# CPJKU/beat_this

Hardware: NVIDIA H100
Metric: clips/sec (30 s audio->beats, final0) (higher is better)
Workload: dtype f16

## Files before the change

beat_this_b200/csrc/kernels_attn.cu:

```cuda
#include <cstdio>

#include "tc_common.cuh"

namespace bt {

constexpr int AT_BQ = 128;
constexpr int AT_BKV = 64;
constexpr int AT_NST = 4;
constexpr int AT_WARPS = 8;
constexpr int AT_THREADS = 32 * (AT_WARPS + 1);
constexpr int AT_SQ = AT_BQ * 64;
constexpr int AT_SKV = AT_BKV * 64;
constexpr int AT_SMEM = 1024 + AT_SQ + AT_NST * 2 * AT_SKV + 128;

constexpr uint32_t AT_POLY_MASK = 0x52u;

__device__ __forceinline__ uint32_t sw64_off(int r, int c) {
  return static_cast<uint32_t>(r * 64 + ((c ^ ((r >> 1) & 3)) << 4));
}

__global__ void __launch_bounds__(AT_THREADS, 2)
attn_time_kernel(const __grid_constant__ CUtensorMap tmQ, const __grid_constant__ CUtensorMap tmKV,
                 const float* __restrict__ gates, h16* __restrict__ out, int L, int heads,
                 const ChunkSrc* __restrict__ chunks, int seqs_per_chunk) {
  extern __shared__ uint8_t smem_raw[];
  const uint32_t sbase = (smem_u32(smem_raw) + 1023u) & ~1023u;
  const uint32_t sQ = sbase;
  const uint32_t sK = sQ + AT_SQ;
  const uint32_t sV = sK + AT_NST * AT_SKV;
  const uint32_t bar_q = sV + AT_NST * AT_SKV;
  const uint32_t full = bar_q + 8;
  const uint32_t empty = full + 8 * AT_NST;

  const int warp = threadIdx.x >> 5, lane = threadIdx.x & 31;
  const int q0 = blockIdx.x * AT_BQ;
  const int h = blockIdx.y;
  const int seq = blockIdx.z;
  const int C = heads * 32;
  const int Lk = chunks ? chunks[seq / seqs_per_chunk].len : L;
  const int nkv = ceil_div(Lk, AT_BKV);

  if (threadIdx.x == 0) {
    mbar_init(bar_q, 1);
    for (int i = 0; i < AT_NST; ++i) {
      mbar_init(full + 8 * i, 1);
      mbar_init(empty + 8 * i, AT_WARPS);
    }
    fence_barrier_init();
  }
  __syncthreads();

  if (warp == AT_WARPS) {
    if (lane == 0) {
      tma_prefetch_desc(&tmQ);
      tma_prefetch_desc(&tmKV);
      mbar_expect_tx(bar_q, AT_SQ);
      tma_load_3d(sQ, &tmQ, bar_q, h * 32, q0, seq);
      for (int j = 0; j < nkv; ++j) {
        const int st = j % AT_NST;
        if (j >= AT_NST) mbar_wait(empty + 8 * st, ((j / AT_NST) - 1) & 1);
        mbar_expect_tx(full + 8 * st, 2 * AT_SKV);
        tma_load_3d(sK + st * AT_SKV, &tmKV, full + 8 * st, C + h * 32, j * AT_BKV, seq);
        tma_load_3d(sV + st * AT_SKV, &tmKV, full + 8 * st, 2 * C + h * 32, j * AT_BKV, seq);
      }
    }
    return;
  }

  const int r0 = warp * 16;
  mbar_wait(bar_q, 0);
  uint32_t qa[2][4];
#pragma unroll
  for (int ks = 0; ks < 2; ++ks) ldmatrix_x4(sQ + sw64_off(r0 + (lane & 15), 2 * ks + (lane >> 4)), qa[ks]);

  float o[4][4];
#pragma unroll
  for (int d = 0; d < 4; ++d) o[d][0] = o[d][1] = o[d][2] = o[d][3] = 0.f;
  float m_run[2] = {-INFINITY, -INFINITY}, l_run[2] = {0.f, 0.f};
  for (int j = 0; j < nkv; ++j) {
    const int st = j % AT_NST;
    mbar_wait(full + 8 * st, (j / AT_NST) & 1);
    const uint32_t kb = sK + st * AT_SKV, vb = sV + st * AT_SKV;
    float s[8][4];
#pragma unroll
    for (int nb = 0; nb < 8; ++nb) {
      s[nb][0] = s[nb][1] = s[nb][2] = s[nb][3] = 0.f;
      uint32_t kf[4];
      ldmatrix_x4(kb + sw64_off(nb * 8 + (lane & 7), lane >> 3), kf);
      mma_16816(s[nb], qa[0], kf[0], kf[1]);
      mma_16816(s[nb], qa[1], kf[2], kf[3]);
    }
    if (j == nkv - 1) {
      const int lim = Lk - j * AT_BKV;
#pragma unroll
      for (int nb = 0; nb < 8; ++nb) {
        const int key = nb * 8 + 2 * (lane & 3);
        if (key >= lim) s[nb][0] = s[nb][2] = -INFINITY;
        if (key + 1 >= lim) s[nb][1] = s[nb][3] = -INFINITY;
      }
    }
    float mx[2] = {-INFINITY, -INFINITY};
#pragma unroll
    for (int nb = 0; nb < 8; ++nb) {
      mx[0] = fmaxf(mx[0], fmaxf(s[nb][0], s[nb][1]));
      mx[1] = fmaxf(mx[1], fmaxf(s[nb][2], s[nb][3]));
    }
    float mref[2], alpha[2];
#pragma unroll
    for (int r = 0; r < 2; ++r) {
      mx[r] = fmaxf(mx[r], __shfl_xor_sync(0xffffffffu, mx[r], 1));
      mx[r] = fmaxf(mx[r], __shfl_xor_sync(0xffffffffu, mx[r], 2));
      mref[r] = fmaxf(m_run[r], mx[r]);
      alpha[r] = ex2_approx(m_run[r] - mref[r]);
      m_run[r] = mref[r];
      l_run[r] *= alpha[r];
    }
#pragma unroll
    for (int d = 0; d < 4; ++d) {
      o[d][0] *= alpha[0]; o[d][1] *= alpha[0];
      o[d][2] *= alpha[1]; o[d][3] *= alpha[1];
    }
    uint32_t pa[4][4];
#pragma unroll
    for (int nb = 0; nb < 8; ++nb) {
      float p[4];
#pragma unroll
      for (int i = 0; i < 4; ++i) {
        const float x = s[nb][i] - mref[i >> 1];
        p[i] = ((AT_POLY_MASK >> nb) & 1u) ? ex2_poly(x) : ex2_approx(x);
      }
      l_run[0] += p[0] + p[1];
      l_run[1] += p[2] + p[3];
      pa[nb >> 1][(nb & 1) * 2] = pack_h16x2(p[0], p[1]);
      pa[nb >> 1][(nb & 1) * 2 + 1] = pack_h16x2(p[2], p[3]);
    }
#pragma unroll
    for (int kk = 0; kk < 4; ++kk) {
      const int key = kk * 16 + (lane & 7) + ((lane >> 3) & 1) * 8;
#pragma unroll
      for (int dp = 0; dp < 2; ++dp) {
        uint32_t vf[4];
        ldmatrix_x4_trans(vb + sw64_off(key, 2 * dp + (lane >> 4)), vf);
        mma_16816(o[2 * dp], pa[kk], vf[0], vf[1]);
        mma_16816(o[2 * dp + 1], pa[kk], vf[2], vf[3]);
      }
    }
    __syncwarp();
    if (lane == 0) mbar_arrive(empty + 8 * st);
  }
#pragma unroll
  for (int r = 0; r < 2; ++r) {
    l_run[r] += __shfl_xor_sync(0xffffffffu, l_run[r], 1);
    l_run[r] += __shfl_xor_sync(0xffffffffu, l_run[r], 2);
  }
#pragma unroll
  for (int r = 0; r < 2; ++r) {
    const int q = q0 + r0 + (lane >> 2) + 8 * r;
    if (q < L) {
      const int64_t m = static_cast<int64_t>(seq) * L + q;
      const float gsc = gates[m * heads + h] / l_run[r];
      h16* dst = out + m * C + h * 32 + 2 * (lane & 3);
#pragma unroll
      for (int d = 0; d < 4; ++d)
        *reinterpret_cast<uint32_t*>(dst + 8 * d) = pack_h16x2(o[d][2 * r] * gsc, o[d][2 * r + 1] * gsc);
    }
  }
}

struct TcAttnPlan {
  CUtensorMap tmQ;
  CUtensorMap tmKV;
  int seqs, L, heads;
};

TcAttnPlan* tc_attn_plan_create(const void* qkv, int seqs, int L, int heads, char* err, int errlen) {
  TcAttnPlan* p = new TcAttnPlan();
  p->seqs = seqs; p->L = L; p->heads = heads;
  const int C = heads * 32;
  const uint64_t dims[3] = {static_cast<uint64_t>(3 * C), static_cast<uint64_t>(L), static_cast<uint64_t>(seqs)};
  const uint64_t strides[2] = {static_cast<uint64_t>(3 * C) * 2, static_cast<uint64_t>(L) * 3 * C * 2};
  const uint32_t box_q[3] = {32, AT_BQ, 1};
  const uint32_t box_kv[3] = {32, AT_BKV, 1};
  if (!make_tmap(&p->tmQ, qkv, 3, dims, strides, box_q, 64, err, errlen) ||
      !make_tmap(&p->tmKV, qkv, 3, dims, strides, box_kv, 64, err, errlen)) {
    delete p;
    return nullptr;
  }
  return p;
}
void tc_attn_plan_destroy(TcAttnPlan* p) { delete p; }

void launch_attn_time_tc(const TcAttnPlan* p, const float* gates, void* out, cudaStream_t st, const ChunkSrc* chunks,
                         int seqs_per_chunk) {
  dim3 grid(ceil_div(p->L, AT_BQ), p->heads, p->seqs);
  attn_time_kernel<<<grid, AT_THREADS, AT_SMEM, st>>>(p->tmQ, p->tmKV, gates, reinterpret_cast<h16*>(out), p->L, p->heads,
                                                      chunks, seqs_per_chunk);
}

int tc_init_attn(char* err, int errlen) {
  const cudaError_t r = cudaFuncSetAttribute(attn_time_kernel, cudaFuncAttributeMaxDynamicSharedMemorySize, AT_SMEM);
  if (r != cudaSuccess) {
    snprintf(err, errlen, "cudaFuncSetAttribute(attn_time_kernel) failed: %s", cudaGetErrorString(r));
    return -1;
  }
  return 0;
}

}
```

Baseline: 746.4.

## Fold TMA producer into consumer thread and peel masked last KV tile

Removes the dedicated producer warp. Thread 0 of the first consumer warp issues the initial KV prefetches, then refills each stage one iteration late after waiting on the empty barrier. The loop body moves into a templated tile function: the boundary mask applies only to the peeled final tile, the running max uses a tree reduction, ldmatrix addresses are precomputed per lane, and output rescaling is skipped when alpha is one for the whole warp. Dropping the producer warp frees warp slots and registers, but refill latency now sits on a compute warp's critical path and that warp may stall waiting for the others to release a stage.

```diff
diff --git a/beat_this_b200/csrc/kernels_attn.cu b/beat_this_b200/csrc/kernels_attn.cu
--- a/beat_this_b200/csrc/kernels_attn.cu
+++ b/beat_this_b200/csrc/kernels_attn.cu
@@ -8,7 +8,7 @@
 constexpr int AT_BKV = 64;
 constexpr int AT_NST = 4;
 constexpr int AT_WARPS = 8;
-constexpr int AT_THREADS = 32 * (AT_WARPS + 1);
+constexpr int AT_THREADS = 32 * AT_WARPS;
 constexpr int AT_SQ = AT_BQ * 64;
 constexpr int AT_SKV = AT_BKV * 64;
 constexpr int AT_SMEM = 1024 + AT_SQ + AT_NST * 2 * AT_SKV + 128;
@@ -17,6 +17,86 @@
 
 __device__ __forceinline__ uint32_t sw64_off(int r, int c) {
   return static_cast<uint32_t>(r * 64 + ((c ^ ((r >> 1) & 3)) << 4));
+}
+
+__device__ __forceinline__ uint32_t opaque_u32(uint32_t v) {
+  asm volatile("" : "+r"(v));
+  return v;
+}
+
+template <bool kMasked>
+__device__ __forceinline__ void attn_time_tile(const uint32_t (&qa)[2][4], uint32_t kaddr, uint32_t vaddr, int key0,
+                                               int lim, float (&o)[4][4], float (&m_run)[2], float (&l_run)[2]) {
+  float s[8][4];
+#pragma unroll
+  for (int nb = 0; nb < 8; ++nb) {
+    s[nb][0] = s[nb][1] = s[nb][2] = s[nb][3] = 0.f;
+    uint32_t kf[4];
+    ldmatrix_x4(kaddr + nb * 8 * 64, kf);
+    mma_16816(s[nb], qa[0], kf[0], kf[1]);
+    mma_16816(s[nb], qa[1], kf[2], kf[3]);
+  }
+  if constexpr (kMasked) {
+#pragma unroll
+    for (int nb = 0; nb < 8; ++nb) {
+      const int key = nb * 8 + key0;
+      if (key >= lim) s[nb][0] = s[nb][2] = -INFINITY;
+      if (key + 1 >= lim) s[nb][1] = s[nb][3] = -INFINITY;
+    }
+  }
+  float mref[2], alpha[2];
+#pragma unroll
+  for (int r = 0; r < 2; ++r) {
+    float t[8];
+#pragma unroll
+    for (int nb = 0; nb < 8; ++nb) t[nb] = fmaxf(s[nb][2 * r], s[nb][2 * r + 1]);
+#pragma unroll
+    for (int w = 4; w > 0; w >>= 1)
+#pragma unroll
+      for (int i = 0; i < w; ++i) t[i] = fmaxf(t[i], t[i + w]);
+    float mx = fmaxf(t[0], __shfl_xor_sync(0xffffffffu, t[0], 1));
+    mx = fmaxf(mx, __shfl_xor_sync(0xffffffffu, mx, 2));
+    mref[r] = fmaxf(m_run[r], mx);
+    alpha[r] = ex2_approx(m_run[r] - mref[r]);
+    m_run[r] = mref[r];
+  }
+  if (!__all_sync(0xffffffffu, alpha[0] == 1.f && alpha[1] == 1.f)) {
+#pragma unroll
+    for (int d = 0; d < 4; ++d) {
+      o[d][0] *= alpha[0]; o[d][1] *= alpha[0];
+      o[d][2] *= alpha[1]; o[d][3] *= alpha[1];
+    }
+  }
+#pragma unroll
+  for (int kk = 0; kk < 4; ++kk) {
+    uint32_t pa[4];
+#pragma unroll
+    for (int h = 0; h < 2; ++h) {
+      const int nb = 2 * kk + h;
+      float p[4];
+#pragma unroll
+      for (int i = 0; i < 4; ++i) {
+        const float x = s[nb][i] - mref[i >> 1];
+        p[i] = ((AT_POLY_MASK >> nb) & 1u) ? ex2_poly(x) : ex2_approx(x);
+      }
+      if (nb == 0) {
+        l_run[0] = fmaf(l_run[0], alpha[0], p[0] + p[1]);
+        l_run[1] = fmaf(l_run[1], alpha[1], p[2] + p[3]);
+      } else {
+        l_run[0] += p[0] + p[1];
+        l_run[1] += p[2] + p[3];
+      }
+      pa[2 * h] = pack_h16x2(p[0], p[1]);
+      pa[2 * h + 1] = pack_h16x2(p[2], p[3]);
+    }
+#pragma unroll
+    for (int dp = 0; dp < 2; ++dp) {
+      uint32_t vf[4];
+      ldmatrix_x4_trans((vaddr ^ (dp * 32)) + kk * 16 * 64, vf);
+      mma_16816(o[2 * dp], pa, vf[0], vf[1]);
+      mma_16816(o[2 * dp + 1], pa, vf[2], vf[3]);
+    }
+  }
 }
 
 __global__ void __launch_bounds__(AT_THREADS, 2)
@@ -39,115 +119,59 @@
   const int C = heads * 32;
   const int Lk = chunks ? chunks[seq / seqs_per_chunk].len : L;
   const int nkv = ceil_div(Lk, AT_BKV);
-
-  if (threadIdx.x == 0) {
+  const bool producer = threadIdx.x == 0;
+  auto load_kv = [&](int t) {
+    const int st = t % AT_NST;
+    mbar_expect_tx(full + 8 * st, 2 * AT_SKV);
+    tma_load_3d(sK + st * AT_SKV, &tmKV, full + 8 * st, C + h * 32, t * AT_BKV, seq);
+    tma_load_3d(sV + st * AT_SKV, &tmKV, full + 8 * st, 2 * C + h * 32, t * AT_BKV, seq);
+  };
+
+  if (producer) {
     mbar_init(bar_q, 1);
     for (int i = 0; i < AT_NST; ++i) {
       mbar_init(full + 8 * i, 1);
       mbar_init(empty + 8 * i, AT_WARPS);
     }
     fence_barrier_init();
+    tma_prefetch_desc(&tmQ);
+    tma_prefetch_desc(&tmKV);
+    mbar_expect_tx(bar_q, AT_SQ);
+    tma_load_3d(sQ, &tmQ, bar_q, h * 32, q0, seq);
+    for (int t = 0; t < AT_NST && t < nkv; ++t) load_kv(t);
   }
   __syncthreads();
-
-  if (warp == AT_WARPS) {
-    if (lane == 0) {
-      tma_prefetch_desc(&tmQ);
-      tma_prefetch_desc(&tmKV);
-      mbar_expect_tx(bar_q, AT_SQ);
-      tma_load_3d(sQ, &tmQ, bar_q, h * 32, q0, seq);
-      for (int j = 0; j < nkv; ++j) {
-        const int st = j % AT_NST;
-        if (j >= AT_NST) mbar_wait(empty + 8 * st, ((j / AT_NST) - 1) & 1);
-        mbar_expect_tx(full + 8 * st, 2 * AT_SKV);
-        tma_load_3d(sK + st * AT_SKV, &tmKV, full + 8 * st, C + h * 32, j * AT_BKV, seq);
-        tma_load_3d(sV + st * AT_SKV, &tmKV, full + 8 * st, 2 * C + h * 32, j * AT_BKV, seq);
-      }
-    }
-    return;
-  }
 
   const int r0 = warp * 16;
   mbar_wait(bar_q, 0);
   uint32_t qa[2][4];
 #pragma unroll
   for (int ks = 0; ks < 2; ++ks) ldmatrix_x4(sQ + sw64_off(r0 + (lane & 15), 2 * ks + (lane >> 4)), qa[ks]);
+  const uint32_t kaddr = opaque_u32(sK + sw64_off(lane & 7, lane >> 3));
+  const uint32_t vaddr = opaque_u32(sV + sw64_off(lane & 15, lane >> 4));
+  const int key0 = 2 * (lane & 3);
 
   float o[4][4];
 #pragma unroll
   for (int d = 0; d < 4; ++d) o[d][0] = o[d][1] = o[d][2] = o[d][3] = 0.f;
   float m_run[2] = {-INFINITY, -INFINITY}, l_run[2] = {0.f, 0.f};
-  for (int j = 0; j < nkv; ++j) {
-    const int st = j % AT_NST;
+  const uint32_t nrefill = opaque_u32(producer && nkv > AT_NST ? nkv - AT_NST : 0);
+  const int nsteady = static_cast<int>(opaque_u32(nkv - 1));
+  for (int j = 0; j < nsteady; ++j) {
+    const uint32_t st = j % AT_NST, so = st * AT_SKV;
     mbar_wait(full + 8 * st, (j / AT_NST) & 1);
-    const uint32_t kb = sK + st * AT_SKV, vb = sV + st * AT_SKV;
-    float s[8][4];
-#pragma unroll
-    for (int nb = 0; nb < 8; ++nb) {
-      s[nb][0] = s[nb][1] = s[nb][2] = s[nb][3] = 0.f;
-      uint32_t kf[4];
-      ldmatrix_x4(kb + sw64_off(nb * 8 + (lane & 7), lane >> 3), kf);
-      mma_16816(s[nb], qa[0], kf[0], kf[1]);
-      mma_16816(s[nb], qa[1], kf[2], kf[3]);
-    }
-    if (j == nkv - 1) {
-      const int lim = Lk - j * AT_BKV;
-#pragma unroll
-      for (int nb = 0; nb < 8; ++nb) {
-        const int key = nb * 8 + 2 * (lane & 3);
-        if (key >= lim) s[nb][0] = s[nb][2] = -INFINITY;
-        if (key + 1 >= lim) s[nb][1] = s[nb][3] = -INFINITY;
-      }
-    }
-    float mx[2] = {-INFINITY, -INFINITY};
-#pragma unroll
-    for (int nb = 0; nb < 8; ++nb) {
-      mx[0] = fmaxf(mx[0], fmaxf(s[nb][0], s[nb][1]));
-      mx[1] = fmaxf(mx[1], fmaxf(s[nb][2], s[nb][3]));
-    }
-    float mref[2], alpha[2];
-#pragma unroll
-    for (int r = 0; r < 2; ++r) {
-      mx[r] = fmaxf(mx[r], __shfl_xor_sync(0xffffffffu, mx[r], 1));
-      mx[r] = fmaxf(mx[r], __shfl_xor_sync(0xffffffffu, mx[r], 2));
-      mref[r] = fmaxf(m_run[r], mx[r]);
-      alpha[r] = ex2_approx(m_run[r] - mref[r]);
-      m_run[r] = mref[r];
-      l_run[r] *= alpha[r];
-    }
-#pragma unroll
-    for (int d = 0; d < 4; ++d) {
-      o[d][0] *= alpha[0]; o[d][1] *= alpha[0];
-      o[d][2] *= alpha[1]; o[d][3] *= alpha[1];
-    }
-    uint32_t pa[4][4];
-#pragma unroll
-    for (int nb = 0; nb < 8; ++nb) {
-      float p[4];
-#pragma unroll
-      for (int i = 0; i < 4; ++i) {
-        const float x = s[nb][i] - mref[i >> 1];
-        p[i] = ((AT_POLY_MASK >> nb) & 1u) ? ex2_poly(x) : ex2_approx(x);
-      }
-      l_run[0] += p[0] + p[1];
-      l_run[1] += p[2] + p[3];
-      pa[nb >> 1][(nb & 1) * 2] = pack_h16x2(p[0], p[1]);
-      pa[nb >> 1][(nb & 1) * 2 + 1] = pack_h16x2(p[2], p[3]);
-    }
-#pragma unroll
-    for (int kk = 0; kk < 4; ++kk) {
-      const int key = kk * 16 + (lane & 7) + ((lane >> 3) & 1) * 8;
-#pragma unroll
-      for (int dp = 0; dp < 2; ++dp) {
-        uint32_t vf[4];
-        ldmatrix_x4_trans(vb + sw64_off(key, 2 * dp + (lane >> 4)), vf);
-        mma_16816(o[2 * dp], pa[kk], vf[0], vf[1]);
-        mma_16816(o[2 * dp + 1], pa[kk], vf[2], vf[3]);
-      }
-    }
-    __syncwarp();
+    attn_time_tile<false>(qa, kaddr + so, vaddr + so, key0, 0, o, m_run, l_run);
+    if (static_cast<uint32_t>(j - 1) < nrefill) {
+      const int t = j + AT_NST - 1;
+      mbar_wait(empty + 8 * (t % AT_NST), ((t / AT_NST) - 1) & 1);
+      load_kv(t);
+    }
     if (lane == 0) mbar_arrive(empty + 8 * st);
   }
+  const uint32_t st = nsteady % AT_NST, parity = (nsteady / AT_NST) & 1;
+  mbar_wait(full + 8 * st, parity);
+  const uint32_t so = st * AT_SKV;
+  attn_time_tile<true>(qa, kaddr + so, vaddr + so, key0, Lk - nsteady * AT_BKV, o, m_run, l_run);
 #pragma unroll
   for (int r = 0; r < 2; ++r) {
     l_run[r] += __shfl_xor_sync(0xffffffffu, l_run[r], 1);
```

Result: faster. 766.2 (median of 6 runs) (+2.7%).

## Give each attention warp two query row blocks and drop the producer warp

Applied to the files above, without the earlier changes.

The time-attention kernel now runs 4 warps, each handling two 16-row query blocks, so every K and V ldmatrix fragment feeds twice as many MMAs. The dedicated TMA producer warp is removed: thread 0 issues the initial stages and refills the ring inline, waiting on the previous stage's empty barrier. The last-tile masking is split into a compile-time specialised step, shared-memory addresses are precomputed, and launch bounds target 3 blocks per SM. This raises register pressure per thread, and refilling from a consumer thread can stall that warp's compute.

```diff
diff --git a/beat_this_b200/csrc/kernels_attn.cu b/beat_this_b200/csrc/kernels_attn.cu
--- a/beat_this_b200/csrc/kernels_attn.cu
+++ b/beat_this_b200/csrc/kernels_attn.cu
@@ -1,4 +1,5 @@
 #include <cstdio>
+#include <type_traits>
 
 #include "tc_common.cuh"
 
@@ -7,11 +8,13 @@
 constexpr int AT_BQ = 128;
 constexpr int AT_BKV = 64;
 constexpr int AT_NST = 4;
-constexpr int AT_WARPS = 8;
-constexpr int AT_THREADS = 32 * (AT_WARPS + 1);
+constexpr int AT_WARPS = 4;
+constexpr int AT_RB = 2;
+constexpr int AT_THREADS = 32 * AT_WARPS;
 constexpr int AT_SQ = AT_BQ * 64;
 constexpr int AT_SKV = AT_BKV * 64;
 constexpr int AT_SMEM = 1024 + AT_SQ + AT_NST * 2 * AT_SKV + 128;
+static_assert(AT_BQ == AT_WARPS * AT_RB * 16, "every query row of the tile belongs to one row block");
 
 constexpr uint32_t AT_POLY_MASK = 0x52u;
 
@@ -19,7 +22,7 @@
   return static_cast<uint32_t>(r * 64 + ((c ^ ((r >> 1) & 3)) << 4));
 }
 
-__global__ void __launch_bounds__(AT_THREADS, 2)
+__global__ void __launch_bounds__(AT_THREADS, 3)
 attn_time_kernel(const __grid_constant__ CUtensorMap tmQ, const __grid_constant__ CUtensorMap tmKV,
                  const float* __restrict__ gates, h16* __restrict__ out, int L, int heads,
                  const ChunkSrc* __restrict__ chunks, int seqs_per_chunk) {
@@ -50,121 +53,163 @@
   }
   __syncthreads();
 
-  if (warp == AT_WARPS) {
-    if (lane == 0) {
-      tma_prefetch_desc(&tmQ);
-      tma_prefetch_desc(&tmKV);
-      mbar_expect_tx(bar_q, AT_SQ);
-      tma_load_3d(sQ, &tmQ, bar_q, h * 32, q0, seq);
-      for (int j = 0; j < nkv; ++j) {
-        const int st = j % AT_NST;
-        if (j >= AT_NST) mbar_wait(empty + 8 * st, ((j / AT_NST) - 1) & 1);
-        mbar_expect_tx(full + 8 * st, 2 * AT_SKV);
-        tma_load_3d(sK + st * AT_SKV, &tmKV, full + 8 * st, C + h * 32, j * AT_BKV, seq);
-        tma_load_3d(sV + st * AT_SKV, &tmKV, full + 8 * st, 2 * C + h * 32, j * AT_BKV, seq);
-      }
-    }
-    return;
-  }
-
-  const int r0 = warp * 16;
+  auto load_tile = [&](int t) {
+    const int st = t % AT_NST;
+    mbar_expect_tx(full + 8 * st, 2 * AT_SKV);
+    tma_load_3d(sK + st * AT_SKV, &tmKV, full + 8 * st, C + h * 32, t * AT_BKV, seq);
+    tma_load_3d(sV + st * AT_SKV, &tmKV, full + 8 * st, 2 * C + h * 32, t * AT_BKV, seq);
+  };
+  if (threadIdx.x == 0) {
+    tma_prefetch_desc(&tmQ);
+    tma_prefetch_desc(&tmKV);
+    mbar_expect_tx(bar_q, AT_SQ);
+    tma_load_3d(sQ, &tmQ, bar_q, h * 32, q0, seq);
+    for (int t = 0; t < nkv && t < AT_NST; ++t) load_tile(t);
+  }
+
+  const int r0 = warp * (AT_RB * 16);
   mbar_wait(bar_q, 0);
-  uint32_t qa[2][4];
-#pragma unroll
-  for (int ks = 0; ks < 2; ++ks) ldmatrix_x4(sQ + sw64_off(r0 + (lane & 15), 2 * ks + (lane >> 4)), qa[ks]);
-
-  float o[4][4];
-#pragma unroll
-  for (int d = 0; d < 4; ++d) o[d][0] = o[d][1] = o[d][2] = o[d][3] = 0.f;
-  float m_run[2] = {-INFINITY, -INFINITY}, l_run[2] = {0.f, 0.f};
-  for (int j = 0; j < nkv; ++j) {
-    const int st = j % AT_NST;
-    mbar_wait(full + 8 * st, (j / AT_NST) & 1);
-    const uint32_t kb = sK + st * AT_SKV, vb = sV + st * AT_SKV;
-    float s[8][4];
+
+  uint32_t qa[AT_RB][2][4];
+#pragma unroll
+  for (int b = 0; b < AT_RB; ++b)
+#pragma unroll
+    for (int ks = 0; ks < 2; ++ks)
+      ldmatrix_x4(sQ + sw64_off(r0 + 16 * b + (lane & 15), 2 * ks + (lane >> 4)), qa[b][ks]);
+
+  const uint32_t k_addr0 = sK + sw64_off(lane & 7, lane >> 3);
+  const uint32_t v_addr0[2] = {sV + sw64_off(lane & 15, lane >> 4), sV + sw64_off(lane & 15, 2 + (lane >> 4))};
+  const int key_lane = 2 * (lane & 3);
+
+  float o[AT_RB][4][4];
+#pragma unroll
+  for (int b = 0; b < AT_RB; ++b)
+#pragma unroll
+    for (int d = 0; d < 4; ++d) o[b][d][0] = o[b][d][1] = o[b][d][2] = o[b][d][3] = 0.f;
+  float m_run[AT_RB][2], l_run[AT_RB][2];
+#pragma unroll
+  for (int b = 0; b < AT_RB; ++b) m_run[b][0] = m_run[b][1] = -INFINITY, l_run[b][0] = l_run[b][1] = 0.f;
+  auto kv_step = [&](uint32_t stage, uint32_t phase, auto last, int lim) {
+    mbar_wait(full + stage / (AT_SKV / 8), phase);
+    const uint32_t ka = k_addr0 + stage, va0 = v_addr0[0] + stage, va1 = v_addr0[1] + stage;
+    float s[AT_RB][8][4];
 #pragma unroll
     for (int nb = 0; nb < 8; ++nb) {
-      s[nb][0] = s[nb][1] = s[nb][2] = s[nb][3] = 0.f;
       uint32_t kf[4];
-      ldmatrix_x4(kb + sw64_off(nb * 8 + (lane & 7), lane >> 3), kf);
-      mma_16816(s[nb], qa[0], kf[0], kf[1]);
-      mma_16816(s[nb], qa[1], kf[2], kf[3]);
-    }
-    if (j == nkv - 1) {
-      const int lim = Lk - j * AT_BKV;
+      ldmatrix_x4(ka + nb * 512, kf);
+#pragma unroll
+      for (int b = 0; b < AT_RB; ++b) {
+        s[b][nb][0] = s[b][nb][1] = s[b][nb][2] = s[b][nb][3] = 0.f;
+        mma_16816(s[b][nb], qa[b][0], kf[0], kf[1]);
+        mma_16816(s[b][nb], qa[b][1], kf[2], kf[3]);
+      }
+    }
+    if constexpr (decltype(last)::value) {
 #pragma unroll
       for (int nb = 0; nb < 8; ++nb) {
-        const int key = nb * 8 + 2 * (lane & 3);
-        if (key >= lim) s[nb][0] = s[nb][2] = -INFINITY;
-        if (key + 1 >= lim) s[nb][1] = s[nb][3] = -INFINITY;
-      }
-    }
-    float mx[2] = {-INFINITY, -INFINITY};
-#pragma unroll
-    for (int nb = 0; nb < 8; ++nb) {
-      mx[0] = fmaxf(mx[0], fmaxf(s[nb][0], s[nb][1]));
-      mx[1] = fmaxf(mx[1], fmaxf(s[nb][2], s[nb][3]));
-    }
-    float mref[2], alpha[2];
-#pragma unroll
-    for (int r = 0; r < 2; ++r) {
-      mx[r] = fmaxf(mx[r], __shfl_xor_sync(0xffffffffu, mx[r], 1));
-      mx[r] = fmaxf(mx[r], __shfl_xor_sync(0xffffffffu, mx[r], 2));
-      mref[r] = fmaxf(m_run[r], mx[r]);
-      alpha[r] = ex2_approx(m_run[r] - mref[r]);
-      m_run[r] = mref[r];
-      l_run[r] *= alpha[r];
-    }
-#pragma unroll
-    for (int d = 0; d < 4; ++d) {
-      o[d][0] *= alpha[0]; o[d][1] *= alpha[0];
-      o[d][2] *= alpha[1]; o[d][3] *= alpha[1];
-    }
-    uint32_t pa[4][4];
-#pragma unroll
-    for (int nb = 0; nb < 8; ++nb) {
-      float p[4];
-#pragma unroll
-      for (int i = 0; i < 4; ++i) {
-        const float x = s[nb][i] - mref[i >> 1];
-        p[i] = ((AT_POLY_MASK >> nb) & 1u) ? ex2_poly(x) : ex2_approx(x);
-      }
-      l_run[0] += p[0] + p[1];
-      l_run[1] += p[2] + p[3];
-      pa[nb >> 1][(nb & 1) * 2] = pack_h16x2(p[0], p[1]);
-      pa[nb >> 1][(nb & 1) * 2 + 1] = pack_h16x2(p[2], p[3]);
-    }
+        const int key = nb * 8 + key_lane;
+#pragma unroll
+        for (int b = 0; b < AT_RB; ++b) {
+          if (key >= lim) s[b][nb][0] = s[b][nb][2] = -INFINITY;
+          if (key + 1 >= lim) s[b][nb][1] = s[b][nb][3] = -INFINITY;
+        }
+      }
+    }
+    float mref[AT_RB][2];
+#pragma unroll
+    for (int b = 0; b < AT_RB; ++b) {
+      float mx[2];
+#pragma unroll
+      for (int r = 0; r < 2; ++r) {
+        float t[8];
+#pragma unroll
+        for (int nb = 0; nb < 8; ++nb) t[nb] = fmaxf(s[b][nb][2 * r], s[b][nb][2 * r + 1]);
+#pragma unroll
+        for (int w = 4; w > 0; w >>= 1)
+#pragma unroll
+          for (int i = 0; i < w; ++i) t[i] = fmaxf(t[i], t[i + w]);
+        mx[r] = t[0];
+      }
+      float alpha[2];
+#pragma unroll
+      for (int r = 0; r < 2; ++r) {
+        mx[r] = fmaxf(mx[r], __shfl_xor_sync(0xffffffffu, mx[r], 1));
+        mx[r] = fmaxf(mx[r], __shfl_xor_sync(0xffffffffu, mx[r], 2));
+        mref[b][r] = fmaxf(m_run[b][r], mx[r]);
+        alpha[r] = ex2_approx(m_run[b][r] - mref[b][r]);
+        m_run[b][r] = mref[b][r];
+        l_run[b][r] *= alpha[r];
+      }
+#pragma unroll
+      for (int d = 0; d < 4; ++d) {
+        o[b][d][0] *= alpha[0]; o[b][d][1] *= alpha[0];
+        o[b][d][2] *= alpha[1]; o[b][d][3] *= alpha[1];
+      }
+    }
+    uint32_t pa[AT_RB][4][4];
+#pragma unroll
+    for (int b = 0; b < AT_RB; ++b)
+#pragma unroll
+      for (int nb = 0; nb < 8; ++nb) {
+        float p[4];
+#pragma unroll
+        for (int i = 0; i < 4; ++i) {
+          const float x = s[b][nb][i] - mref[b][i >> 1];
+          p[i] = ((AT_POLY_MASK >> nb) & 1u) ? ex2_poly(x) : ex2_approx(x);
+        }
+        l_run[b][0] += p[0] + p[1];
+        l_run[b][1] += p[2] + p[3];
+        pa[b][nb >> 1][(nb & 1) * 2] = pack_h16x2(p[0], p[1]);
+        pa[b][nb >> 1][(nb & 1) * 2 + 1] = pack_h16x2(p[2], p[3]);
+      }
 #pragma unroll
     for (int kk = 0; kk < 4; ++kk) {
-      const int key = kk * 16 + (lane & 7) + ((lane >> 3) & 1) * 8;
 #pragma unroll
       for (int dp = 0; dp < 2; ++dp) {
         uint32_t vf[4];
-        ldmatrix_x4_trans(vb + sw64_off(key, 2 * dp + (lane >> 4)), vf);
-        mma_16816(o[2 * dp], pa[kk], vf[0], vf[1]);
-        mma_16816(o[2 * dp + 1], pa[kk], vf[2], vf[3]);
+        ldmatrix_x4_trans((dp ? va1 : va0) + kk * 1024, vf);
+#pragma unroll
+        for (int b = 0; b < AT_RB; ++b) {
+          mma_16816(o[b][2 * dp], pa[b][kk], vf[0], vf[1]);
+          mma_16816(o[b][2 * dp + 1], pa[b][kk], vf[2], vf[3]);
+        }
       }
     }
     __syncwarp();
-    if (lane == 0) mbar_arrive(empty + 8 * st);
-  }
-#pragma unroll
-  for (int r = 0; r < 2; ++r) {
-    l_run[r] += __shfl_xor_sync(0xffffffffu, l_run[r], 1);
-    l_run[r] += __shfl_xor_sync(0xffffffffu, l_run[r], 2);
-  }
-#pragma unroll
-  for (int r = 0; r < 2; ++r) {
-    const int q = q0 + r0 + (lane >> 2) + 8 * r;
-    if (q < L) {
-      const int64_t m = static_cast<int64_t>(seq) * L + q;
-      const float gsc = gates[m * heads + h] / l_run[r];
-      h16* dst = out + m * C + h * 32 + 2 * (lane & 3);
-#pragma unroll
-      for (int d = 0; d < 4; ++d)
-        *reinterpret_cast<uint32_t*>(dst + 8 * d) = pack_h16x2(o[d][2 * r] * gsc, o[d][2 * r + 1] * gsc);
-    }
-  }
+    if (lane == 0) mbar_arrive(empty + stage / (AT_SKV / 8));
+  };
+  uint32_t stage = 0, phase = 0;
+  for (int j = 0; j < nkv - 1; ++j) {
+    if (threadIdx.x == 0 && j > 0 && j + AT_NST - 1 < nkv) {
+      mbar_wait(empty + 8 * ((j - 1) % AT_NST), ((j - 1) / AT_NST) & 1);
+      load_tile(j + AT_NST - 1);
+    }
+    kv_step(stage, phase, std::false_type{}, 0);
+    stage += AT_SKV;
+    if (stage == AT_NST * AT_SKV) stage = 0, phase ^= 1;
+  }
+  if (nkv > 0) kv_step(stage, phase, std::true_type{}, Lk - (nkv - 1) * AT_BKV);
+#pragma unroll
+  for (int b = 0; b < AT_RB; ++b)
+#pragma unroll
+    for (int r = 0; r < 2; ++r) {
+      l_run[b][r] += __shfl_xor_sync(0xffffffffu, l_run[b][r], 1);
+      l_run[b][r] += __shfl_xor_sync(0xffffffffu, l_run[b][r], 2);
+    }
+#pragma unroll
+  for (int b = 0; b < AT_RB; ++b)
+#pragma unroll
+    for (int r = 0; r < 2; ++r) {
+      const int q = q0 + r0 + 16 * b + (lane >> 2) + 8 * r;
+      if (q < L) {
+        const int64_t m = static_cast<int64_t>(seq) * L + q;
+        const float gsc = gates[m * heads + h] / l_run[b][r];
+        h16* dst = out + m * C + h * 32 + 2 * (lane & 3);
+#pragma unroll
+        for (int d = 0; d < 4; ++d)
+          *reinterpret_cast<uint32_t*>(dst + 8 * d) = pack_h16x2(o[b][d][2 * r] * gsc, o[b][d][2 * r + 1] * gsc);
+      }
+    }
 }
 
 struct TcAttnPlan {
```

Result: faster. 758.0 before, 804.3 after, median of 6 (+6.1%).
